# itmanager85/real-time-opencl-raytracer

Hardware: AMD Instinct MI355X
Metric: Mrays/sec (primary+1 shadow) @1080p, 1M-tri SAH BVH; 1/2/4/8 GPU (higher is better)
Workload: dtype f32

## Files before the change

### real-time-opencl-raytracer_amd/csrc/rt_kernel_body.inc

```
namespace RTK_NS {
using rtk::DevScene;
using rtk::Frame;
using rtk::Outputs;
using rtk::Stack;
using rtk::leaf_range;
using rtk::leaf_bytes;
using rtk::kLeafBit;
using rtk::kRefError;
using rtk::kStackSize;
using rtk::kTmin;
using rtk::kLdsStack;
using rtk::QRay;
using rtk::WQ;
using rtk::tile_epilogue;

__device__ __forceinline__ float xdiv(float a, float d, float y) {
    const float q = a * y;
    const float r = __builtin_fmaf(-q, d, a);
    return __builtin_fmaf(r, y, q);
}
__device__ __forceinline__ bool axis_ok(float o, float d) {
    const float ad = fabsf(d), ao = fabsf(o);
    const bool o_ok = ao == 0.0f || (ao >= 0x1p-66f && ao <= 0x1p60f);
    if (kMath == 2) return o_ok && (ad == 0.0f || ad >= 0x1p-126f);
    return ad == 0.0f || (ad >= 0x1p-64f && ad <= 2.0f && o_ok);
}
__device__ __forceinline__ bool fast_div_ok(const Ray& r) {
    return axis_ok(r.ori.x, r.dir.x) && axis_ok(r.ori.y, r.dir.y) && axis_ok(r.ori.z, r.dir.z);
}
__device__ __forceinline__ F3 slab_recip(const Ray& r) {
    if (kMath == 2) return F3{rcp_(r.dir.x), rcp_(r.dir.y), rcp_(r.dir.z)};
    return r.inv_dir;
}

typedef float v2f __attribute__((ext_vector_type(2)));
template <int S> __device__ __forceinline__ v2f pk_sub(v2f b, v2f O) {
    v2f a;
    if (S) asm("v_pk_add_f32 %0, %1, %2 op_sel:[0,1] op_sel_hi:[1,1] neg_lo:[0,1] neg_hi:[0,1]" : "=v"(a) : "v"(b), "v"(O));
    else   asm("v_pk_add_f32 %0, %1, %2 op_sel_hi:[1,0] neg_lo:[0,1] neg_hi:[0,1]" : "=v"(a) : "v"(b), "v"(O));
    return a;
}
template <int S> __device__ __forceinline__ v2f pk_mulb(v2f a, v2f Y) {
    v2f q;
    if (S) asm("v_pk_mul_f32 %0, %1, %2 op_sel:[0,1] op_sel_hi:[1,1]" : "=v"(q) : "v"(a), "v"(Y));
    else   asm("v_pk_mul_f32 %0, %1, %2 op_sel_hi:[1,0]" : "=v"(q) : "v"(a), "v"(Y));
    return q;
}
template <int S> __device__ __forceinline__ v2f pk_res(v2f q, v2f D, v2f a) {
    v2f r;
    if (S) asm("v_pk_fma_f32 %0, %1, %2, %3 op_sel:[0,1,0] op_sel_hi:[1,1,1] neg_lo:[1,0,0] neg_hi:[1,0,0]" : "=v"(r) : "v"(q), "v"(D), "v"(a));
    else   asm("v_pk_fma_f32 %0, %1, %2, %3 op_sel_hi:[1,0,1] neg_lo:[1,0,0] neg_hi:[1,0,0]" : "=v"(r) : "v"(q), "v"(D), "v"(a));
    return r;
}
template <int S> __device__ __forceinline__ v2f pk_cor(v2f r, v2f Y, v2f q) {
    v2f o;
    if (S) asm("v_pk_fma_f32 %0, %1, %2, %3 op_sel:[0,1,0] op_sel_hi:[1,1,1]" : "=v"(o) : "v"(r), "v"(Y), "v"(q));
    else   asm("v_pk_fma_f32 %0, %1, %2, %3 op_sel_hi:[1,0,1]" : "=v"(o) : "v"(r), "v"(Y), "v"(q));
    return o;
}
__device__ __forceinline__ v2f pk_pick(bool dzero, v2f res, v2f q) {
    res.x = dzero ? q.x : res.x;
    res.y = dzero ? q.y : res.y;
    return res;
}
__device__ __forceinline__ float min_(float a, float b) { float r; asm("v_min_f32 %0, %1, %2" : "=v"(r) : "v"(a), "v"(b)); return r; }
__device__ __forceinline__ float max_(float a, float b) { float r; asm("v_max_f32 %0, %1, %2" : "=v"(r) : "v"(a), "v"(b)); return r; }
__device__ __forceinline__ float min3_(float a, float b, float c) {
    float r; asm("v_min3_f32 %0, %1, %2, %3" : "=v"(r) : "v"(a), "v"(b), "v"(c)); return r;
}
__device__ __forceinline__ float max3_(float a, float b, float c) {
    float r; asm("v_max3_f32 %0, %1, %2, %3" : "=v"(r) : "v"(a), "v"(b), "v"(c)); return r;
}
struct RayPk {
    v2f oxy, ozdz, yxy, dxy, yz;
    bool zx, zy, zz;
};
__device__ __forceinline__ RayPk ray_pk(const F3& o, const F3& d, const F3& y) {
    float ox = o.x, oy = o.y, oz = o.z, dx = d.x, dy = d.y, dz = d.z, yx = y.x, yy = y.y, yz = y.z;
    asm("" : "+v"(ox), "+v"(oy), "+v"(oz), "+v"(dx), "+v"(dy), "+v"(dz), "+v"(yx), "+v"(yy), "+v"(yz));
    return RayPk{v2f{ox, oy}, v2f{oz, dz}, v2f{yx, yy}, v2f{dx, dy}, v2f{yz, yz}, d.x == 0.0f, d.y == 0.0f,
                 d.z == 0.0f};
}
template <bool ZERO = true, int OCT = -1>
__device__ __forceinline__ void slab2_pk(const float4& q0, const float4& q1, const float4& q2, const RayPk& R,
                                         float& n0, float& f0, float& n1, float& f1) {
    const v2f a0 = pk_sub<0>(v2f{q0.x, q0.y}, R.oxy), a1 = pk_sub<0>(v2f{q0.z, q0.w}, R.oxy);
    const v2f a2 = pk_sub<1>(v2f{q1.x, q1.y}, R.oxy), a3 = pk_sub<1>(v2f{q1.z, q1.w}, R.oxy);
    const v2f a4 = pk_sub<0>(v2f{q2.x, q2.y}, R.ozdz), a5 = pk_sub<0>(v2f{q2.z, q2.w}, R.ozdz);
    const v2f m0 = pk_mulb<0>(a0, R.yxy), m1 = pk_mulb<0>(a1, R.yxy);
    const v2f m2 = pk_mulb<1>(a2, R.yxy), m3 = pk_mulb<1>(a3, R.yxy);
    const v2f m4 = pk_mulb<0>(a4, R.yz), m5 = pk_mulb<0>(a5, R.yz);
    v2f ax, bx, ay, by, az, bz;
    if (kMath == 2) {
        ax = m0; bx = m1; ay = m2; by = m3; az = m4; bz = m5;
    } else {
        const v2f r0 = pk_res<0>(m0, R.dxy, a0), r1 = pk_res<0>(m1, R.dxy, a1);
        const v2f r2 = pk_res<1>(m2, R.dxy, a2), r3 = pk_res<1>(m3, R.dxy, a3);
        const v2f r4 = pk_res<1>(m4, R.ozdz, a4), r5 = pk_res<1>(m5, R.ozdz, a5);
        ax = pk_cor<0>(r0, R.yxy, m0); bx = pk_cor<0>(r1, R.yxy, m1);
        ay = pk_cor<1>(r2, R.yxy, m2); by = pk_cor<1>(r3, R.yxy, m3);
        az = pk_cor<0>(r4, R.yz, m4); bz = pk_cor<0>(r5, R.yz, m5);
        if (ZERO) {
            ax = pk_pick(R.zx, ax, m0); bx = pk_pick(R.zx, bx, m1);
            ay = pk_pick(R.zy, ay, m2); by = pk_pick(R.zy, by, m3);
            az = pk_pick(R.zz, az, m4); bz = pk_pick(R.zz, bz, m5);
        }
    }
    if (OCT >= 0) {
        static_assert(OCT < 0 || !ZERO, "an octant loop has no zero direction component");
        const v2f nx = (OCT & 1) ? bx : ax, fx = (OCT & 1) ? ax : bx;
        const v2f ny = (OCT & 2) ? by : ay, fy = (OCT & 2) ? ay : by;
        const v2f nz = (OCT & 4) ? bz : az, fz = (OCT & 4) ? az : bz;
        n0 = max3_(nx.x, ny.x, nz.x);
        f0 = min3_(fx.x, fy.x, fz.x);
        n1 = max3_(nx.y, ny.y, nz.y);
        f1 = min3_(fx.y, fy.y, fz.y);
        return;
    }
    n0 = max3_(min_(ax.x, bx.x), min_(ay.x, by.x), min_(az.x, bz.x));
    f0 = min3_(max_(ax.x, bx.x), max_(ay.x, by.x), max_(az.x, bz.x));
    n1 = max3_(min_(ax.y, bx.y), min_(ay.y, by.y), min_(az.y, bz.y));
    f1 = min3_(max_(ax.y, bx.y), max_(ay.y, by.y), max_(az.y, bz.y));
}
__device__ __forceinline__ void slab2_div(const float4& q0, const float4& q1, const float4& q2, const F3& o,
                                          const F3& d, float& n0, float& f0, float& n1, float& f1) {
    const v2f ax = v2f{div_(q0.x - o.x, d.x), div_(q0.y - o.x, d.x)}, bx = v2f{div_(q0.z - o.x, d.x), div_(q0.w - o.x, d.x)};
    const v2f ay = v2f{div_(q1.x - o.y, d.y), div_(q1.y - o.y, d.y)}, by = v2f{div_(q1.z - o.y, d.y), div_(q1.w - o.y, d.y)};
    const v2f az = v2f{div_(q2.x - o.z, d.z), div_(q2.y - o.z, d.z)}, bz = v2f{div_(q2.z - o.z, d.z), div_(q2.w - o.z, d.z)};
    n0 = fmaxf(fmaxf(fminf(ax.x, bx.x), fminf(ay.x, by.x)), fminf(az.x, bz.x));
    f0 = fminf(fminf(fmaxf(ax.x, bx.x), fmaxf(ay.x, by.x)), fmaxf(az.x, bz.x));
    n1 = fmaxf(fmaxf(fminf(ax.y, bx.y), fminf(ay.y, by.y)), fminf(az.y, bz.y));
    f1 = fminf(fminf(fmaxf(ax.y, bx.y), fmaxf(ay.y, by.y)), fmaxf(az.y, bz.y));
}

struct Trav {
    uint32_t cur, nxt;
    int sc;
    int result;
    float tHit;
};

template <bool CLOSEST>
__device__ __forceinline__ void trav_step(const DevScene& S, const Ray& ray, const F3& y, bool fast, Trav& T,
                                          const Stack& st, bool& overflow) {
    const F3 o = ray.ori, d = ray.dir;
    while (T.sc > 0 && !(T.cur & kLeafBit)) {
        if (T.cur == kRefError) {
            T.result = -1;
            T.sc = 0;
            break;
        }
        const float4* np = S.wnodes + (size_t)T.cur * 4;
        const float4 q0 = np[0], q1 = np[1], q2 = np[2], q3 = np[3];
        float n0, f0, n1, f1;
        if (fast) slab2_pk<true>(q0, q1, q2, ray_pk(o, d, y), n0, f0, n1, f1);
        else slab2_div(q0, q1, q2, o, d, n0, f0, n1, f1);
        const bool i0 = (n0 <= f0) && (f0 >= kTmin) && (n0 <= T.tHit);
        const bool i1 = (n1 <= f1) && (f1 >= kTmin) && (n1 <= T.tHit);
        const uint32_t r0 = __float_as_uint(q3.x), r1 = __float_as_uint(q3.y);
        if (i0 && i1) {
            if (T.sc >= kStackSize) {
                overflow = true;
                T.result = -1;
                T.sc = 0;
                break;
            }
            const bool swap = n0 > n1;
            if (T.sc >= 2) st.put(T.sc - 2, T.nxt);
            T.nxt = swap ? r0 : r1;
            T.cur = swap ? r1 : r0;
            ++T.sc;
        } else if (i0 || i1) {
            T.cur = i0 ? r0 : r1;
        } else {
            --T.sc;
            T.cur = T.nxt;
            if (T.sc >= 2) T.nxt = st.get(T.sc - 2);
        }
    }
    if (T.sc > 0) {
        int off, cnt;
        leaf_range(S, T.cur, off, cnt);
        bool stop = false;
        for (int i = 0; i < cnt; ++i) {
            const float4* tp = tri_rec(S, off + i);
            const float4 a0 = tp[0], a1 = tp[1], a2 = tp[2];
            const F3 e2 = F3{a2.x, a2.y, a2.z};
            const float t = ray_tri(ray, F3{a0.x, a0.y, a0.z}, F3{a1.x, a1.y, a1.z}, e2);
            if (t < T.tHit && t > kTmin) {
                T.tHit = t;
                T.result = __float_as_int(a0.w);
                if (!CLOSEST) { stop = true; break; }
            }
        }
        if (stop) {
            T.sc = 0;
        } else {
            --T.sc;
            T.cur = T.nxt;
            if (T.sc >= 2) T.nxt = st.get(T.sc - 2);
        }
    }
}

template <bool CLOSEST>
__device__ int traverse(const DevScene& S, const Ray& ray, float& tHit, const Stack& st, bool& overflow) {
    Trav T;
    T.cur = S.root;
    T.nxt = 0;
    T.sc = 1;
    T.result = -1;
    T.tHit = tHit;
    const bool fast = S.fast_div && fast_div_ok(ray);
    const F3 y = slab_recip(ray);
    do {
        trav_step<CLOSEST>(S, ray, y, fast, T, st, overflow);
    } while (T.sc > 0);
    tHit = T.tHit;
    return T.result;
}

constexpr bool kOctLoops = kMath == 2;
constexpr uint32_t kStackBase = 0x80000000u - (uint32_t)(kLdsStack + 1) * 256u, kStackDone = 0u;
typedef __attribute__((address_space(3))) uint32_t lds_u32;
__device__ __forceinline__ uint32_t lds_get(int a) { return *(lds_u32*)(uintptr_t)(uint32_t)a; }
__device__ __forceinline__ void lds_put(int a, uint32_t v) { *(lds_u32*)(uintptr_t)(uint32_t)a = v; }
template <bool GUARD> __device__ __forceinline__ int slot_get(int col0, uint32_t sb) {
    return GUARD ? (int)((uint32_t)col0 - (kStackBase + rtk::kLdsGuard * 256u) + sb)
                 : col0 + max((int)(sb - kStackBase) - 512, 0);
}
template <bool GUARD> __device__ __forceinline__ int slot_put(int get_at, int col0, uint32_t sb) {
    return GUARD ? get_at + 256 : col0 + max((int)(sb - kStackBase) - 256, 0);
}

template <int MODE, int OCT = -1>
__device__ __forceinline__ void inner_step(const float4& q0, const float4& q1, const float4& q2, float2 refs,
                                           const RayPk& rp, float th, uint32_t popped, int put_at,
                                           uint32_t& cur, uint32_t& nxt, uint32_t& sb) {
    float n0, f0, n1, f1;
    if (MODE == 2) {
        slab2_div(q0, q1, q2, F3{rp.oxy.x, rp.oxy.y, rp.ozdz.x}, F3{rp.dxy.x, rp.dxy.y, rp.ozdz.y}, n0, f0, n1, f1);
    } else {
        slab2_pk<MODE == 1, MODE == 0 ? OCT : -1>(q0, q1, q2, rp, n0, f0, n1, f1);
    }
    const bool i0 = (n0 <= min_(f0, th)) && (f0 >= kTmin);
    const bool i1 = (n1 <= min_(f1, th)) && (f1 >= kTmin);
    const uint32_t r0 = __float_as_uint(refs.x), r1 = __float_as_uint(refs.y);
    lds_put(put_at, nxt);
    const bool both = i0 && i1, none = !i0 && !i1;
    const bool swap = n0 > n1;
    const uint32_t nearr = swap ? r1 : r0, farr = swap ? r0 : r1, one = i0 ? r0 : r1;
    const uint32_t ncur = both ? nearr : (none ? nxt : one);
    nxt = both ? farr : (none ? popped : nxt);
    cur = ncur;
    sb += (both ? 256u : 0u) - (none ? 256u : 0u);
}

__device__ __forceinline__ Ray ray_of(const RayPk& rp, const F3& inv) {
    Ray r;
    r.ori = F3{rp.oxy.x, rp.oxy.y, rp.ozdz.x};
    r.dir = F3{rp.dxy.x, rp.dxy.y, rp.ozdz.y};
    r.inv_dir = inv;
    return r;
}

__device__ __forceinline__ float4 rec_load4(__amdgpu_buffer_rsrc_t r, uint32_t off) {
    const auto v = __builtin_amdgcn_raw_buffer_load_b128(r, (int)off, 0, 0);
    return make_float4(__uint_as_float(v[0]), __uint_as_float(v[1]), __uint_as_float(v[2]), __uint_as_float(v[3]));
}
__device__ __forceinline__ float2 rec_load2(__amdgpu_buffer_rsrc_t r, uint32_t off) {
    const auto v = __builtin_amdgcn_raw_buffer_load_b64(r, (int)off, 0, 0);
    return make_float2(__uint_as_float(v[0]), __uint_as_float(v[1]));
}

template <bool CLOSEST, int MODE, int TR, bool SEL = false, bool GUARD = true, int OCT = -1>
__device__ __forceinline__ bool traverse_ifif(const DevScene& S, Ray& ray_io, float& tHit, const Stack& st,
                                              int& result) {
    const int col0 = (int)(uint32_t)(uintptr_t)(lds_u32*)st.lds;
    const RayPk rp = ray_pk(ray_io.ori, ray_io.dir, slab_recip(ray_io));
    const F3 inv_keep = F3{rp.yxy.x, rp.yxy.y, rp.yz.x};
    uint32_t cur = S.root, nxt = 0;
    uint32_t sb = kStackBase;
    int res = -1;
    float th = tHit;
    uint32_t tk = 0, tend = 0;
    const __amdgpu_buffer_rsrc_t recs =
        __builtin_amdgcn_make_buffer_rsrc((void*)S.wnodes, (short)0, (int)S.rec_bytes, 0x00020000);
    typedef unsigned int su4 __attribute__((ext_vector_type(4)));
    typedef unsigned int su2 __attribute__((ext_vector_type(2)));
    typedef const __attribute__((address_space(4))) su4 csu4;
    typedef const __attribute__((address_space(4))) su2 csu2;
    if (TR == 2 && CLOSEST) rtk::timeline_mark(st.fc, 6);
    while ((int)sb >= (int)kStackBase) {
        const uint32_t c0 = __builtin_amdgcn_readfirstlane(cur);
        if (__builtin_amdgcn_ballot_w64(cur != c0) != 0 || (c0 & kLeafBit)) break;
        const int at = slot_get<GUARD>(col0, sb);
        const uint32_t popped = lds_get(at);
        if (TR == 1) rtk::fetch_count(st.fc, false, cur, false);
        if (TR == 2) rtk::timeline_step(st.fc, CLOSEST ? 1 : 3);
        csu4* rec = (csu4*)((const char*)S.wnodes + ((size_t)c0 << 6));
        const su4 u0 = rec[0], u1 = rec[1], u2 = rec[2];
        const su2 u3 = *(csu2*)(rec + 3);
        const float4 q0 = make_float4(__uint_as_float(u0.x), __uint_as_float(u0.y), __uint_as_float(u0.z), __uint_as_float(u0.w));
        const float4 q1 = make_float4(__uint_as_float(u1.x), __uint_as_float(u1.y), __uint_as_float(u1.z), __uint_as_float(u1.w));
        const float4 q2 = make_float4(__uint_as_float(u2.x), __uint_as_float(u2.y), __uint_as_float(u2.z), __uint_as_float(u2.w));
        const float2 q3 = make_float2(__uint_as_float(u3.x), __uint_as_float(u3.y));
        inner_step<MODE, OCT>(q0, q1, q2, q3, rp, th, popped, slot_put<GUARD>(at, col0, sb), cur, nxt, sb);
    }
    if (TR == 2 && CLOSEST) rtk::timeline_mark(st.fc, 7);
    while ((int)sb >= (int)kStackBase) {
        const bool leaf = (cur & kLeafBit) != 0;
        if (leaf && tk >= tend) leaf_bytes(S, cur, tk, tend);
        const int at = slot_get<GUARD>(col0, sb);
        const uint32_t popped = lds_get(at);
        if (TR == 1) rtk::fetch_count(st.fc, leaf, leaf ? (0x80000000u | tk) : cur);
        if (TR == 2) rtk::timeline_step(st.fc, CLOSEST ? 0 : 2);
        uint32_t off;
        if (SEL) {
            asm("v_cndmask_b32 %0, %1, %2, %3" : "=v"(off) : "v"(cur << 6), "v"(tk), "s"(__builtin_amdgcn_ballot_w64(leaf)));
        } else {
            off = leaf ? tk : cur << 6;
        }
        uint32_t t_issue = 0;
        if (TR == 2 && RTK_TL_SPLIT) t_issue = (uint32_t)__builtin_amdgcn_s_memrealtime();
        const float4 q0 = rec_load4(recs, off), q1 = rec_load4(recs, off + 16u), q2 = rec_load4(recs, off + 32u);
        float2 q3 = make_float2(0.0f, 0.0f);
        if (!leaf) q3 = rec_load2(recs, off + 48u);
        asm volatile("" ::: "memory");
        if (TR == 2 && RTK_TL_SPLIT) {
            asm volatile("" ::"v"(q0.x), "v"(q1.x), "v"(q2.x), "v"(q3.x));
            rtk::timeline_wait(st.fc, CLOSEST ? 0 : 1, (uint32_t)__builtin_amdgcn_s_memrealtime() - t_issue);
        }
        if (!leaf) {
            inner_step<MODE, OCT>(q0, q1, q2, q3, rp, th, popped, slot_put<GUARD>(at, col0, sb), cur, nxt, sb);
        } else {
            const F3 e2 = F3{q2.x, q2.y, q2.z};
            const float t = ray_tri(ray_of(rp, inv_keep), F3{q0.x, q0.y, q0.z}, F3{q1.x, q1.y, q1.z}, e2);
            const bool hit = t < th && t > kTmin && tk < tend;
            th = hit ? t : th;
            res = hit ? __float_as_int(q0.w) : res;
            tk += 48u;
            const bool pop = tk >= tend;
            cur = pop ? nxt : cur;
            nxt = pop ? popped : nxt;
            sb -= pop ? 256u : 0u;
            if (!CLOSEST) sb = hit ? kStackDone : sb;
        }
    }
    tHit = th;
    result = res;
    ray_io = ray_of(rp, inv_keep);
    return (int)sb >= 0;
}

template <bool CLOSEST, int TR>
__device__ __forceinline__ void variant_count(const Stack& st, int which) {
    if (TR == 1 && (uint32_t)(threadIdx.x & 63u) == (uint32_t)__builtin_ctzll(__builtin_amdgcn_read_exec()))
        atomicAdd(st.vc + (CLOSEST ? 0 : 9) + which, 1ull);
}
template <bool CLOSEST, int TR, bool SEL = false, bool GUARD = true, bool OCTS = false>
__device__ __forceinline__ bool traverse_fast(const DevScene& S, Ray& ray, float& tHit, const Stack& st,
                                              int& result) {
    if (!S.fast_div || __builtin_amdgcn_ballot_w64(!fast_div_ok(ray))) {
        variant_count<CLOSEST, TR>(st, 0);
        return traverse_ifif<CLOSEST, 2, TR, SEL, GUARD>(S, ray, tHit, st, result);
    }
    if (kMath != 2) {
        const bool z = ray.dir.x == 0.0f || ray.dir.y == 0.0f || ray.dir.z == 0.0f;
        if (__builtin_amdgcn_ballot_w64(z)) {
            variant_count<CLOSEST, TR>(st, 0);
            return traverse_ifif<CLOSEST, 1, TR, SEL, GUARD>(S, ray, tHit, st, result);
        }
    }
    if (OCTS) {
        const bool z = ray.dir.x == 0.0f || ray.dir.y == 0.0f || ray.dir.z == 0.0f;
        const uint64_t act = __builtin_amdgcn_read_exec();
        const uint64_t sx = __builtin_amdgcn_ballot_w64(ray.dir.x < 0.0f), sy = __builtin_amdgcn_ballot_w64(ray.dir.y < 0.0f),
                       sz = __builtin_amdgcn_ballot_w64(ray.dir.z < 0.0f);
        const bool uniform = (sx == 0 || sx == act) && (sy == 0 || sy == act) && (sz == 0 || sz == act);
        const int oct = (sx ? 1 : 0) | (sy ? 2 : 0) | (sz ? 4 : 0);
        if (__builtin_amdgcn_ballot_w64(z) == 0 && uniform) {
            variant_count<CLOSEST, TR>(st, 1 + oct);
            switch (oct) {
                case 0: return traverse_ifif<CLOSEST, 0, TR, SEL, GUARD, 0>(S, ray, tHit, st, result);
                case 1: return traverse_ifif<CLOSEST, 0, TR, SEL, GUARD, 1>(S, ray, tHit, st, result);
                case 2: return traverse_ifif<CLOSEST, 0, TR, SEL, GUARD, 2>(S, ray, tHit, st, result);
                case 3: return traverse_ifif<CLOSEST, 0, TR, SEL, GUARD, 3>(S, ray, tHit, st, result);
                case 4: return traverse_ifif<CLOSEST, 0, TR, SEL, GUARD, 4>(S, ray, tHit, st, result);
                case 5: return traverse_ifif<CLOSEST, 0, TR, SEL, GUARD, 5>(S, ray, tHit, st, result);
                case 6: return traverse_ifif<CLOSEST, 0, TR, SEL, GUARD, 6>(S, ray, tHit, st, result);
                default: return traverse_ifif<CLOSEST, 0, TR, SEL, GUARD, 7>(S, ray, tHit, st, result);
            }
        }
    }
    variant_count<CLOSEST, TR>(st, 0);
    return traverse_ifif<CLOSEST, 0, TR, SEL, GUARD>(S, ray, tHit, st, result);
}

template <bool CLOSEST, bool FASTONLY, int TR = 0, bool SEL = false, bool GUARD = true, bool OCTS = false>
__device__ __forceinline__ int trace(const DevScene& S, const Outputs& O, Ray& ray, float& t, const Stack& st,
                                     bool& overflow, float t_restart = 4294967296.0f) {
    int hit;
    if (FASTONLY) {
        if (traverse_fast<CLOSEST, TR, SEL, GUARD, OCTS>(S, ray, t, st, hit)) return hit;
        atomicAdd(O.restarts, 1u);
        t = t_restart;
    }
    return traverse<CLOSEST>(S, ray, t, st, overflow);
}


__device__ __forceinline__ Ray primary_ray(const Frame& F, uint32_t x, uint32_t y) {
    const float xf = (float)(((double)x - 0.5) / (double)(float)F.w);
    const float yf = (float)(((double)y - 0.5) / (double)(float)F.h);
    const F3 a = F3{F.a.x, F.a.y, F.a.z}, b = F3{F.b.x, F.b.y, F.b.z}, c = F3{F.c.x, F.c.y, F.c.z};
    const F3 campos = F3{F.campos.x, F.campos.y, F.campos.z};
    const F3 t1 = mad3(a, xf, c);
    const F3 t2 = b * yf;
    const F3 image_pos = t1 + t2;
    return ray_init(image_pos, image_pos - campos);
}

__device__ __forceinline__ bool scene_box_hit(const Frame& F, const Ray& r) {
    return ray_box_scene(F3{F.smin.x, F.smin.y, F.smin.z}, F3{F.smax.x, F.smax.y, F.smax.z}, r.ori, r.inv_dir);
}

__device__ __forceinline__ void shade_hit(const DevScene& S, const Frame& F, const Ray& ray, float tHit, int hit,
                                          F3& rez, F3& hitpoint, F3& normal, F3& L) {
    const F3 light_pos = F3{F.light_pos.x, F.light_pos.y, F.light_pos.z};
    const float4* sp = S.shade + (size_t)(hit / 3) * 7;
    const float4 p0 = sp[0], p1 = sp[1], p2 = sp[2], m0 = sp[3], m1 = sp[4], m2 = sp[5], alb = sp[6];
    const F3 vNew = mad3(ray.dir, tHit - 0.001f, ray.ori);
    normal = normalize(normal_at(vNew, xyz(p0), xyz(p1), xyz(p2), xyz(m0), xyz(m1), xyz(m2)));
    const F3 l1 = normalize(light_pos - vNew);
    const F3 v = normalize(ray.ori - vNew);
    const F3 n = normalize(normal);
    const F3 albedo = xyz(alb);
    const float f0 = 40.0f * (1.0f / 255.0f);
    rez = cook_torrance_ggx(n, l1, v, albedo, f0, 0.5f) * 3.0f;
    rez = rez + F3{0.3f, 0.3f, 0.3f} * albedo;
    hitpoint = vNew;
    L = normalize(light_pos - hitpoint);
}

__device__ __forceinline__ F3 finish_color(F3 color, float shadow_sum, int ray_depth) {
    if (ray_depth >= 1) {
        const float dd = (float)ray_depth;
        color = F3{div_(color.x, dd), div_(color.y, dd), div_(color.z, dd)};
        shadow_sum = div_(shadow_sum, dd);
        return color * shadow_sum;
    }
    return F3{0, 0, 0};
}

__device__ __forceinline__ void park_next(const F3& dir, const F3& normal, const F3& hitpoint, float* next) {
    const F3 refl = reflect(dir, normal);
    const F3 no = mad3(refl, 0.001f, hitpoint);
    next[0] = no.x; next[64] = no.y; next[128] = no.z;
    next[192] = refl.x; next[256] = refl.y; next[320] = refl.z;
}

template <bool FASTONLY, int TR = 0, bool SEL = false, bool GUARD = true, bool OCTS = false>
__device__ __forceinline__ float shadow_coef(const DevScene& S, const Outputs& O, const F3& hitpoint, const F3& L,
                                             const Stack& st, bool& overflow, int& sh) {
    Ray sray = ray_init(mad3(L, 0.001f, hitpoint), L);
    float ts = 4294967296.0f;
    sh = trace<false, FASTONLY, TR, SEL, GUARD, OCTS>(S, O, sray, ts, st, overflow);
    return (sh >= 0 && ts > 0.025f) ? 0.25f : 1.0f;
}

template <bool FASTONLY>
__device__ __forceinline__ void render_pixel(const DevScene& S, const Frame& F, const Outputs& O, int want_aux,
                                             uint32_t x, uint32_t y, uint32_t pix, const Stack& st, float* next) {
    bool overflow = false;
    const int depth = F.depth;
    Ray ray = primary_ray(F, x, y);
    if (want_aux) {
        for (int k = 0; k < depth; ++k) {
            O.hits[((size_t)pix * depth + k) * 2 + 0] = -2;
            O.hits[((size_t)pix * depth + k) * 2 + 1] = -2;
            O.t[(size_t)pix * depth + k] = -1.0f;
        }
    }
    float tHit = 4294967296.0f;
    bool cont = scene_box_hit(F, ray);
    F3 color = F3{0, 0, 0};
// ... 316 lines not shown
```

### real-time-opencl-raytracer_amd/csrc/rt_render.hip

```cpp
#include <hip/hip_runtime.h>
#include <hip/hip_ext.h>

#include <algorithm>
#include <array>
#include <atomic>
#include <chrono>
#include <cmath>
#include <condition_variable>
#include <cstdio>
#include <cstdlib>
#include <cstring>
#include <mutex>
#include <string>
#include <thread>
#include <utility>
#include <vector>

#include "rt_abi.h"
#include "rt_records.h"
#include "rt_refit.h"
#include "refit.hpp"
#include "scene_encode.hpp"
#include "rt_lbvh.h"
#include "rt_scene_build.h"
// ... 20 lines not shown
#endif
#ifndef RTK_QUERY_GRID_PCT
#define RTK_QUERY_GRID_PCT 75
#endif
#ifndef RTK_FB_WAVES
#define RTK_FB_WAVES 8
#endif
#ifndef RTK_EXT_EVENTS
#define RTK_EXT_EVENTS 1
#endif
#ifndef RTK_LDS_STACK
#define RTK_LDS_STACK 16
#endif
#ifndef RTK_XFRAME
#define RTK_XFRAME 1
#endif

namespace rtk {

constexpr int kStackSize = 65;
constexpr float kTmin = 0.001f;
using rtrec::kCntEscape;
using rtrec::kLeafBit;
using rtrec::kRefError;
constexpr int kLdsStack = RTK_LDS_STACK;
constexpr int kGlobalStack = 64 - kLdsStack;
constexpr int kLdsGuard = 2;
constexpr int kLdsRows = kLdsGuard + kLdsStack;
constexpr uint32_t kBlockPx = 16;
constexpr uint32_t kBlockThreads = 256;

struct DevScene {
    const float4* __restrict__ wnodes;
    const float4* __restrict__ tris;
    const float4* __restrict__ shade;
    const int2* __restrict__ leaf_table;
    uint32_t tri_off;
    uint32_t rec_bytes;
    uint32_t root;
    uint32_t n_inner;
    int fast_div;
    int clean;
};

__device__ __forceinline__ const float4* tri_rec(const DevScene& S, int k) { return S.tris + (size_t)k * 3; }

struct Frame {
    float3 a, b, c, campos, light_pos, smin, smax;
    uint32_t w, h;
    int32_t depth;
    uint32_t flags;
    int32_t rank, nranks, band_rows;
    uint32_t local_rows;
    uint32_t tiles_x, tiles_y, num_blocks;
    const uint32_t* tile_order;
    uint32_t* tile_cost;
    uint32_t* lpt_next;
    uint32_t* done;
    uint32_t* zero_next;
    uint32_t nzero;
};

struct QRay {
    float4 a, b, c;
};
#ifndef RTK_SORT_SCALE
#define RTK_SORT_SCALE 4
#endif
#ifndef RTK_SORT_SCALE_BATCH
#define RTK_SORT_SCALE_BATCH 8
#endif
#ifndef RTK_CHUNK_SEGS
#define RTK_CHUNK_SEGS 32
#endif
constexpr uint32_t kChunkSegs = RTK_CHUNK_SEGS, kSuperSegs = 1024;
struct WQ {
    const QRay* in;
    const uint32_t* in_count;
    const uint32_t* perm;
    QRay* out;
    uint32_t* seg_cnt;
    uint32_t* chunk_sum;
    uint32_t* super_sum;
    uint32_t seg;
    uint32_t* seg_fill;
    uint32_t* fetch;
    int bounce;
};
constexpr uint32_t kSegRays = 64;

constexpr uint32_t kCursors = 8, kCursorStride = 32;
constexpr size_t kCursorSet = (size_t)kCursors * kCursorStride;
constexpr uint32_t kNoGroup = 0xFFFFFFFFu;
__device__ __forceinline__ uint32_t grab_group(uint32_t* cursors, uint32_t ngroups, uint32_t& home) {
    uint32_t g = kNoGroup, h = home;
    if ((threadIdx.x & 63u) == 0) {
        for (uint32_t k = 0; k < kCursors; ++k) {
            const uint32_t c = (h + k) & (kCursors - 1u);
            const uint32_t gg = c + kCursors * atomicAdd(cursors + c * kCursorStride, 1u);
            if (gg < ngroups) {
                g = gg;
                h = c;
                break;
            }
        }
    }
    home = __builtin_amdgcn_readfirstlane(h);
    return __builtin_amdgcn_readfirstlane(g);
}

struct Query {
    const float4* rays;
    uint2* hits;
    uint32_t n;
    uint32_t* fetch;
};

struct Outputs {
    uint32_t* out;
    int32_t* hits;
    float* t;
    float* rgb;
    uint32_t* gstack;
    unsigned long long* overflow;
    uint32_t* restarts;
    uint64_t local_pixels;
    unsigned long long* fcount;
    uint32_t frame_rows;
    uint32_t* wtime;
};

constexpr int kMaxBatch = RT_MAX_BATCH;
struct BatchCam {
    float4 a, b, c, campos, light_pos;
};
struct BatchCams {
    BatchCam cam[kMaxBatch];
    uint64_t stride;
    uint32_t frame_px;
};

__device__ __forceinline__ void leaf_range(const DevScene& S, uint32_t ref, int& off, int& cnt) {
    uint32_t c = rtrec::ref_count(ref);
    if (c == kCntEscape) {
        int2 e = S.leaf_table[rtrec::ref_offset(ref)];
        off = e.x;
        cnt = e.y;
    } else {
        off = (int)rtrec::ref_offset(ref);
        cnt = (int)c;
    }
}

__device__ __forceinline__ void leaf_bytes(const DevScene& S, uint32_t ref, uint32_t& tk, uint32_t& tend) {
    int off, cnt;
    leaf_range(S, ref, off, cnt);
    tk = S.tri_off + (uint32_t)off * 48u;
    tend = tk + (uint32_t)cnt * 48u;
}

struct Stack {
    uint32_t* lds;
    uint32_t* glb;
    uint64_t gstride;
    uint32_t* fc = nullptr;
    unsigned long long* vc = nullptr;
    __device__ __forceinline__ uint32_t get(int i) const {
        return i < kLdsStack ? lds[i * 64] : glb[(uint64_t)(i - kLdsStack) * gstride];
    }
    __device__ __forceinline__ void put(int i, uint32_t v) const {
        if (i < kLdsStack) lds[i * 64] = v;
        else glb[(uint64_t)(i - kLdsStack) * gstride] = v;
    }
};

constexpr int kFetchCounts = 8, kVariantCounts = 18;
__device__ __forceinline__ void fetch_count(uint32_t* fc, bool leaf, uint32_t id, bool vmem = true) {
    const uint64_t act = __builtin_amdgcn_read_exec();
    const int lane = (int)(threadIdx.x & 63u);
    bool quad_first = true, wave_first = true;
    for (int j = 0; j < 64; ++j) {
        const uint32_t b = (uint32_t)__shfl((int)id, j);
        if (j < lane && ((act >> j) & 1ull) && b == id) {
            wave_first = false;
            if ((j >> 2) == (lane >> 2)) quad_first = false;
        }
    }
    const uint64_t lm = __builtin_amdgcn_ballot_w64(leaf);
    const int t = leaf ? 1 : 0;
    fc[t * 256] += 1u;
    fc[(2 + t) * 256] += (vmem && quad_first) ? 1u : 0u;
    fc[(4 + t) * 256] += wave_first ? 1u : 0u;
    if (lane == (int)__builtin_ctzll(act)) {
        fc[6 * 256] += 1u;
        fc[7 * 256] += (lm != 0 && (act & ~lm) != 0) ? 1u : 0u;
    }
}

__device__ __forceinline__ void fetch_count_flush(const uint32_t* fc_block, unsigned long long* out) {
    __syncthreads();
    if (threadIdx.x < 8) {
        unsigned long long sum = 0;
        for (int i = 0; i < 256; ++i) sum += fc_block[threadIdx.x * 256 + i];
        atomicAdd(out + threadIdx.x, sum);
    }
}

__device__ __forceinline__ uint32_t frame_row(const Frame& F, uint32_t lr) {
    if (F.nranks <= 1) return lr;
    const uint32_t band = lr / (uint32_t)F.band_rows, rib = lr % (uint32_t)F.band_rows;
    return (band * (uint32_t)F.nranks + (uint32_t)F.rank) * (uint32_t)F.band_rows + rib;
}

#ifndef RTK_TL_SPLIT
#define RTK_TL_SPLIT 0
#endif
constexpr uint32_t kTlWords = 12, kTlRecord = 20, kTlLongWait = 25;
__device__ __forceinline__ void timeline_step(uint32_t* c, int which) {
    if ((uint32_t)(threadIdx.x & 63u) == (uint32_t)__builtin_ctzll(__builtin_amdgcn_read_exec())) c[which] += 1u;
}
__device__ __forceinline__ void timeline_wait(uint32_t* c, int which, uint32_t ticks) {
    if ((uint32_t)(threadIdx.x & 63u) == (uint32_t)__builtin_ctzll(__builtin_amdgcn_read_exec())) {
        c[8 + which] += ticks;
        c[10 + which] += ticks >= kTlLongWait ? 1u : 0u;
    }
}
__device__ __forceinline__ void timeline_mark(uint32_t* c, int which) {
    if ((uint32_t)(threadIdx.x & 63u) == (uint32_t)__builtin_ctzll(__builtin_amdgcn_read_exec()))
        c[which] = (uint32_t)__builtin_amdgcn_s_memrealtime();
}
__device__ __forceinline__ void timeline_store(const Outputs& O, uint32_t w, uint32_t t0, uint32_t t1,
                                               const uint32_t* c, uint32_t tag) {
    const uint32_t t2 = (uint32_t)__builtin_amdgcn_s_memrealtime();
    if ((threadIdx.x & 63u) == 0) {
        uint4* r = reinterpret_cast<uint4*>(O.wtime + (size_t)w * kTlRecord);
        r[0] = make_uint4(t0, c[4], c[5], t1);
        r[1] = make_uint4(t2, c[0], c[1], c[2]);
        r[2] = make_uint4(c[3], (uint32_t)__builtin_amdgcn_s_getreg(20 | (15 << 11)),
                          (uint32_t)__builtin_amdgcn_s_getreg(4 | (31 << 11)), tag);
        r[3] = make_uint4(c[6], c[7], 0u, 0u);
        r[4] = make_uint4(c[8], c[9], c[10], c[11]);
    }
}

__device__ __forceinline__ uint32_t block_tile(const Frame& F) { return F.tile_order[blockIdx.x]; }

__device__ __forceinline__ void tile_pixel(const Frame& F, uint32_t tb, int wave, int l, uint32_t& x, uint32_t& lr) {
    const uint32_t tx = tb % F.tiles_x, ty = tb / F.tiles_x;
    const uint32_t lx = (uint32_t)((l & 1) | ((l >> 1) & 2) | ((l >> 2) & 4));
    const uint32_t ly = (uint32_t)(((l >> 1) & 1) | ((l >> 2) & 2) | ((l >> 3) & 4));
    x = tx * kBlockPx + (uint32_t)(wave & 1) * 8u + lx;
    lr = ty * kBlockPx + (uint32_t)(wave >> 1) * 8u + ly;
}

__device__ __forceinline__ void zero_next_counters(const Frame& F) {
    const uint32_t bd = blockDim.x;
    const uint32_t n = gridDim.x * bd;
    for (uint32_t i = blockIdx.x * bd + threadIdx.x; i < F.nzero; i += n) F.zero_next[i] = 0u;
}

__device__ __forceinline__ QRay* seg_slot(QRay* q, uint32_t seg, uint32_t* fill) {
    const uint64_t m = __builtin_amdgcn_ballot_w64(true);
    const int lane = threadIdx.x & 63;
    const int leader = __builtin_ctzll(m);
    uint32_t base = 0;
    if (lane == leader) base = atomicAdd(fill, (uint32_t)__builtin_popcountll(m));
    base = (uint32_t)__shfl((int)base, leader);
    return q + (size_t)seg * kSegRays + base + (uint32_t)__builtin_popcountll(m & ((1ull << lane) - 1ull));
}
__device__ __forceinline__ void seg_close(const WQ& W, uint32_t seg) {
    if ((threadIdx.x & 63u) == 0) {
        const uint32_t c = *W.seg_fill;
        W.seg_cnt[seg] = c;
        if (c) {
            atomicAdd(W.chunk_sum + seg / kChunkSegs, c);
            atomicAdd(W.super_sum + seg / kSuperSegs, c);
        }
        *W.seg_fill = 0u;
    }
}

__device__ __forceinline__ uint32_t lpt_key(uint32_t c) {
    if (c == 0) return 0;
    const uint32_t e = 31u - __builtin_clz(c);
    const uint32_t m = e >= 3 ? (c >> (e - 3)) & 7u : (c << (3 - e)) & 7u;
    return min(255u, e * 8u + m);
}

#ifndef RTK_LPT_VEC
#define RTK_LPT_VEC 1
#endif
constexpr int kEpilogueWords = 8 + 256 + 2 * 256;
static_assert(4 * kLdsStack * 64 >= kEpilogueWords, "tile_epilogue's scratch must fit the blocks' traversal stacks");
constexpr uint32_t kKeyBytes = (4u * kLdsStack * 64u - (uint32_t)kEpilogueWords) * 4u;
typedef unsigned int u32x4 __attribute__((ext_vector_type(4)));
__device__ __forceinline__ void load_costs16(const uint32_t* cost, uint32_t q0, uint32_t nq, u32x4 (&v)[4]) {
    const u32x4* c4 = reinterpret_cast<const u32x4*>(cost);
#pragma unroll
    for (int u = 0; u < 4; ++u) {
        const u32x4* p = c4 + min(q0 + (uint32_t)u * 256u + threadIdx.x, nq - 1u);
        asm volatile("global_load_dwordx4 %0, %1, off sc1" : "=v"(v[u]) : "v"(p) : "memory");
    }
    asm volatile("s_waitcnt vmcnt(0)" : "+v"(v[0]), "+v"(v[1]), "+v"(v[2]), "+v"(v[3]) : : "memory");
}
__device__ void tile_epilogue(const Frame& F, uint32_t tb, uint32_t t_start, uint32_t* scratch) {
    if (!F.tile_cost) return;
    const uint32_t tid = threadIdx.x, lane = tid & 63u, wave = tid >> 6;
    const uint32_t t_end = (uint32_t)__builtin_amdgcn_s_memrealtime();
    __syncthreads();
    if (lane == 0) scratch[wave] = t_end - t_start + 1u;
    __syncthreads();
// ... 2542 lines not shown
```

Before: 15450.

## Add lean traversal path with scalar box math and tolerant uniform loop

For the SEL (and !GUARD) traversal variants, box-slab math in the wave-uniform phase moves to scalar-operand VALU forms, since node data loaded through a uniform address sits in SGPRs. The uniform loop now tolerates inactive lanes by picking the node from the first live lane, and leaf byte offsets are decoded with shift-add instructions. Reading the child refs is deferred until the inner-node branch, which lowers register pressure but gives the load less time to arrive before use. Which kernels actually run the new path depends on which template variants the dispatcher selects.

Result: faster. 16930 (median of 6 runs) (+9.6%).

```diff
diff --git a/real-time-opencl-raytracer_amd/csrc/rt_kernel_body.inc b/real-time-opencl-raytracer_amd/csrc/rt_kernel_body.inc
--- a/real-time-opencl-raytracer_amd/csrc/rt_kernel_body.inc
+++ b/real-time-opencl-raytracer_amd/csrc/rt_kernel_body.inc
@@ -34,14 +34,31 @@
 }
 
 typedef float v2f __attribute__((ext_vector_type(2)));
-template <int S> __device__ __forceinline__ v2f pk_sub(v2f b, v2f O) {
+template <int S, int SB = 0> __device__ __forceinline__ v2f pk_sub(v2f b, v2f O) {
     v2f a;
+    if (SB == 2) {
+        const float o = S ? O.y : O.x;
+        asm("v_sub_f32 %0, %1, %2" : "=v"(a.x) : "s"(b.x), "v"(o));
+        asm("v_sub_f32 %0, %1, %2" : "=v"(a.y) : "s"(b.y), "v"(o));
+        return a;
+    }
+    if (SB == 1) {
+        if (S) asm("v_pk_add_f32 %0, %1, %2 op_sel:[0,1] op_sel_hi:[1,1] neg_lo:[0,1] neg_hi:[0,1]" : "=v"(a) : "s"(b), "v"(O));
+        else   asm("v_pk_add_f32 %0, %1, %2 op_sel_hi:[1,0] neg_lo:[0,1] neg_hi:[0,1]" : "=v"(a) : "s"(b), "v"(O));
+        return a;
+    }
     if (S) asm("v_pk_add_f32 %0, %1, %2 op_sel:[0,1] op_sel_hi:[1,1] neg_lo:[0,1] neg_hi:[0,1]" : "=v"(a) : "v"(b), "v"(O));
     else   asm("v_pk_add_f32 %0, %1, %2 op_sel_hi:[1,0] neg_lo:[0,1] neg_hi:[0,1]" : "=v"(a) : "v"(b), "v"(O));
     return a;
 }
-template <int S> __device__ __forceinline__ v2f pk_mulb(v2f a, v2f Y) {
+template <int S, int SB = 0> __device__ __forceinline__ v2f pk_mulb(v2f a, v2f Y) {
     v2f q;
+    if (SB == 2) {
+        const float y = S ? Y.y : Y.x;
+        asm("v_mul_f32 %0, %1, %2" : "=v"(q.x) : "v"(a.x), "v"(y));
+        asm("v_mul_f32 %0, %1, %2" : "=v"(q.y) : "v"(a.y), "v"(y));
+        return q;
+    }
     if (S) asm("v_pk_mul_f32 %0, %1, %2 op_sel:[0,1] op_sel_hi:[1,1]" : "=v"(q) : "v"(a), "v"(Y));
     else   asm("v_pk_mul_f32 %0, %1, %2 op_sel_hi:[1,0]" : "=v"(q) : "v"(a), "v"(Y));
     return q;
@@ -81,15 +98,15 @@
     return RayPk{v2f{ox, oy}, v2f{oz, dz}, v2f{yx, yy}, v2f{dx, dy}, v2f{yz, yz}, d.x == 0.0f, d.y == 0.0f,
                  d.z == 0.0f};
 }
-template <bool ZERO = true, int OCT = -1>
+template <bool ZERO = true, int OCT = -1, int SB = 0>
 __device__ __forceinline__ void slab2_pk(const float4& q0, const float4& q1, const float4& q2, const RayPk& R,
                                          float& n0, float& f0, float& n1, float& f1) {
-    const v2f a0 = pk_sub<0>(v2f{q0.x, q0.y}, R.oxy), a1 = pk_sub<0>(v2f{q0.z, q0.w}, R.oxy);
-    const v2f a2 = pk_sub<1>(v2f{q1.x, q1.y}, R.oxy), a3 = pk_sub<1>(v2f{q1.z, q1.w}, R.oxy);
-    const v2f a4 = pk_sub<0>(v2f{q2.x, q2.y}, R.ozdz), a5 = pk_sub<0>(v2f{q2.z, q2.w}, R.ozdz);
-    const v2f m0 = pk_mulb<0>(a0, R.yxy), m1 = pk_mulb<0>(a1, R.yxy);
-    const v2f m2 = pk_mulb<1>(a2, R.yxy), m3 = pk_mulb<1>(a3, R.yxy);
-    const v2f m4 = pk_mulb<0>(a4, R.yz), m5 = pk_mulb<0>(a5, R.yz);
+    const v2f a0 = pk_sub<0, SB>(v2f{q0.x, q0.y}, R.oxy), a1 = pk_sub<0, SB>(v2f{q0.z, q0.w}, R.oxy);
+    const v2f a2 = pk_sub<1, SB>(v2f{q1.x, q1.y}, R.oxy), a3 = pk_sub<1, SB>(v2f{q1.z, q1.w}, R.oxy);
+    const v2f a4 = pk_sub<0, SB>(v2f{q2.x, q2.y}, R.ozdz), a5 = pk_sub<0, SB>(v2f{q2.z, q2.w}, R.ozdz);
+    const v2f m0 = pk_mulb<0, SB>(a0, R.yxy), m1 = pk_mulb<0, SB>(a1, R.yxy);
+    const v2f m2 = pk_mulb<1, SB>(a2, R.yxy), m3 = pk_mulb<1, SB>(a3, R.yxy);
+    const v2f m4 = pk_mulb<0, SB>(a4, R.yz), m5 = pk_mulb<0, SB>(a5, R.yz);
     v2f ax, bx, ay, by, az, bz;
     if (kMath == 2) {
         ax = m0; bx = m1; ay = m2; by = m3; az = m4; bz = m5;
@@ -233,7 +250,7 @@
     return GUARD ? get_at + 256 : col0 + max((int)(sb - kStackBase) - 256, 0);
 }
 
-template <int MODE, int OCT = -1>
+template <int MODE, int OCT = -1, int SB = 0>
 __device__ __forceinline__ void inner_step(const float4& q0, const float4& q1, const float4& q2, float2 refs,
                                            const RayPk& rp, float th, uint32_t popped, int put_at,
                                            uint32_t& cur, uint32_t& nxt, uint32_t& sb) {
@@ -241,7 +258,7 @@
     if (MODE == 2) {
         slab2_div(q0, q1, q2, F3{rp.oxy.x, rp.oxy.y, rp.ozdz.x}, F3{rp.dxy.x, rp.dxy.y, rp.ozdz.y}, n0, f0, n1, f1);
     } else {
-        slab2_pk<MODE == 1, MODE == 0 ? OCT : -1>(q0, q1, q2, rp, n0, f0, n1, f1);
+        slab2_pk<MODE == 1, MODE == 0 ? OCT : -1, SB>(q0, q1, q2, rp, n0, f0, n1, f1);
     }
     const bool i0 = (n0 <= min_(f0, th)) && (f0 >= kTmin);
     const bool i1 = (n1 <= min_(f1, th)) && (f1 >= kTmin);
@@ -276,6 +293,8 @@
 template <bool CLOSEST, int MODE, int TR, bool SEL = false, bool GUARD = true, int OCT = -1>
 __device__ __forceinline__ bool traverse_ifif(const DevScene& S, Ray& ray_io, float& tHit, const Stack& st,
                                               int& result) {
+    constexpr bool kLean = SEL, kShiftDecode = SEL || !GUARD;
+    constexpr int kScalarBox = MODE == 2 ? 0 : SEL ? 2 : GUARD ? 0 : 1;
     const int col0 = (int)(uint32_t)(uintptr_t)(lds_u32*)st.lds;
     const RayPk rp = ray_pk(ray_io.ori, ray_io.dir, slab_recip(ray_io));
     const F3 inv_keep = F3{rp.yxy.x, rp.yxy.y, rp.yz.x};
@@ -284,6 +303,8 @@
     int res = -1;
     float th = tHit;
     uint32_t tk = 0, tend = 0;
+    uint32_t tri_off = S.tri_off;
+    if (SEL && kOctLoops) asm("" : "+v"(tri_off));
     const __amdgpu_buffer_rsrc_t recs =
         __builtin_amdgcn_make_buffer_rsrc((void*)S.wnodes, (short)0, (int)S.rec_bytes, 0x00020000);
     typedef unsigned int su4 __attribute__((ext_vector_type(4)));
@@ -291,9 +312,7 @@
     typedef const __attribute__((address_space(4))) su4 csu4;
     typedef const __attribute__((address_space(4))) su2 csu2;
     if (TR == 2 && CLOSEST) rtk::timeline_mark(st.fc, 6);
-    while ((int)sb >= (int)kStackBase) {
-        const uint32_t c0 = __builtin_amdgcn_readfirstlane(cur);
-        if (__builtin_amdgcn_ballot_w64(cur != c0) != 0 || (c0 & kLeafBit)) break;
+    const auto uniform_step = [&](uint32_t c0) __attribute__((always_inline)) {
         const int at = slot_get<GUARD>(col0, sb);
         const uint32_t popped = lds_get(at);
         if (TR == 1) rtk::fetch_count(st.fc, false, cur, false);
@@ -305,33 +324,65 @@
         const float4 q1 = make_float4(__uint_as_float(u1.x), __uint_as_float(u1.y), __uint_as_float(u1.z), __uint_as_float(u1.w));
         const float4 q2 = make_float4(__uint_as_float(u2.x), __uint_as_float(u2.y), __uint_as_float(u2.z), __uint_as_float(u2.w));
         const float2 q3 = make_float2(__uint_as_float(u3.x), __uint_as_float(u3.y));
-        inner_step<MODE, OCT>(q0, q1, q2, q3, rp, th, popped, slot_put<GUARD>(at, col0, sb), cur, nxt, sb);
+        inner_step<MODE, OCT, kScalarBox>(q0, q1, q2, q3, rp, th, popped, slot_put<GUARD>(at, col0, sb), cur, nxt, sb);
+    };
+    if (kLean) {
+        for (;;) {
+            const bool live = (int)sb >= (int)kStackBase;
+            const uint64_t lm = __builtin_amdgcn_ballot_w64(live);
+            if (lm == 0) break;
+            const uint32_t c0 = __builtin_amdgcn_readlane(cur, __builtin_ctzll(lm));
+            if ((__builtin_amdgcn_ballot_w64(cur != (c0 & ~kLeafBit)) & lm) != 0) break;
+            asm volatile("");
+            if (live) uniform_step(c0);
+        }
+    } else {
+        while ((int)sb >= (int)kStackBase) {
+            const uint32_t c0 = __builtin_amdgcn_readfirstlane(cur);
+            if (__builtin_amdgcn_ballot_w64(cur != c0) != 0 || (c0 & kLeafBit)) break;
+            uniform_step(c0);
+        }
     }
     if (TR == 2 && CLOSEST) rtk::timeline_mark(st.fc, 7);
     while ((int)sb >= (int)kStackBase) {
         const bool leaf = (cur & kLeafBit) != 0;
-        if (leaf && tk >= tend) leaf_bytes(S, cur, tk, tend);
+        uint32_t off = 0;
+        const auto select_off = [&]() __attribute__((always_inline)) {
+            if (SEL) {
+                asm("v_cndmask_b32 %0, %1, %2, %3" : "=v"(off) : "v"(cur << 6), "v"(tk), "s"(__builtin_amdgcn_ballot_w64(leaf)));
+            } else {
+                off = leaf ? tk : cur << 6;
+            }
+        };
+        if (kLean) select_off();
+        if (leaf && tk >= tend) {
+            leaf_bytes<kShiftDecode>(S, tri_off, cur, tk, tend);
+            off = tk;
+        }
+        if (!kLean) select_off();
         const int at = slot_get<GUARD>(col0, sb);
         const uint32_t popped = lds_get(at);
         if (TR == 1) rtk::fetch_count(st.fc, leaf, leaf ? (0x80000000u | tk) : cur);
         if (TR == 2) rtk::timeline_step(st.fc, CLOSEST ? 0 : 2);
-        uint32_t off;
-        if (SEL) {
-            asm("v_cndmask_b32 %0, %1, %2, %3" : "=v"(off) : "v"(cur << 6), "v"(tk), "s"(__builtin_amdgcn_ballot_w64(leaf)));
-        } else {
-            off = leaf ? tk : cur << 6;
-        }
         uint32_t t_issue = 0;
         if (TR == 2 && RTK_TL_SPLIT) t_issue = (uint32_t)__builtin_amdgcn_s_memrealtime();
         const float4 q0 = rec_load4(recs, off), q1 = rec_load4(recs, off + 16u), q2 = rec_load4(recs, off + 32u);
-        float2 q3 = make_float2(0.0f, 0.0f);
-        if (!leaf) q3 = rec_load2(recs, off + 48u);
-        asm volatile("" ::: "memory");
+        constexpr bool kRefsEarly = (TR == 2 && RTK_TL_SPLIT) || !kLean;
+        float2 q3;
+        if (kRefsEarly) {
+            q3 = make_float2(0.0f, 0.0f);
+            if (!leaf) q3 = rec_load2(recs, off + 48u);
+            asm volatile("" ::: "memory");
+        }
         if (TR == 2 && RTK_TL_SPLIT) {
             asm volatile("" ::"v"(q0.x), "v"(q1.x), "v"(q2.x), "v"(q3.x));
             rtk::timeline_wait(st.fc, CLOSEST ? 0 : 1, (uint32_t)__builtin_amdgcn_s_memrealtime() - t_issue);
         }
         if (!leaf) {
+            if (!kRefsEarly) {
+                q3 = rec_load2(recs, off + 48u);
+                __builtin_amdgcn_sched_barrier(0);
+            }
             inner_step<MODE, OCT>(q0, q1, q2, q3, rp, th, popped, slot_put<GUARD>(at, col0, sb), cur, nxt, sb);
         } else {
             const F3 e2 = F3{q2.x, q2.y, q2.z};
diff --git a/real-time-opencl-raytracer_amd/csrc/rt_render.hip b/real-time-opencl-raytracer_amd/csrc/rt_render.hip
--- a/real-time-opencl-raytracer_amd/csrc/rt_render.hip
+++ b/real-time-opencl-raytracer_amd/csrc/rt_render.hip
@@ -196,11 +196,20 @@
     }
 }
 
-__device__ __forceinline__ void leaf_bytes(const DevScene& S, uint32_t ref, uint32_t& tk, uint32_t& tend) {
+template <bool SHIFT>
+__device__ __forceinline__ void leaf_bytes(const DevScene& S, uint32_t tri_off, uint32_t ref, uint32_t& tk, uint32_t& tend) {
     int off, cnt;
     leaf_range(S, ref, off, cnt);
-    tk = S.tri_off + (uint32_t)off * 48u;
-    tend = tk + (uint32_t)cnt * 48u;
+    if (!SHIFT) {
+        tk = tri_off + (uint32_t)off * 48u;
+        tend = tk + (uint32_t)cnt * 48u;
+        return;
+    }
+    uint32_t o3, c3;
+    asm("v_lshl_add_u32 %0, %1, 1, %1" : "=v"(o3) : "v"(off));
+    asm("v_lshl_add_u32 %0, %1, 1, %1" : "=v"(c3) : "v"(cnt));
+    asm("v_lshl_add_u32 %0, %1, 4, %2" : "=v"(tk) : "v"(o3), "v"(tri_off));
+    asm("v_lshl_add_u32 %0, %1, 4, %2" : "=v"(tend) : "v"(c3), "v"(tk));
 }
 
 struct Stack {
```
